# zhangyk18/GeoBi-GNN

Hardware: AMD Instinct MI355X
Metric: M-edges/s (fwd+bwd) on Synthetic set (higher is better)
Workload: dtype f32; 1 GPU; Synthetic train, batch=4 meshes (~20k faces each), fwd+bwd [BASELINE.json configs[2]]: per rank 4 noisy icospheres n=32 (F=20480) as one disjoint-union graph, L1/L1 loss, grad all-reduce + Adam step inside the timed region; ONE resident batch replayed every step, its level-0 CSR / reverse-edge index / corner lists / loss weights built in warm-up and cached per mesh (with --full, extra.fresh_batch:; meshes_per_rank=4, edges_per_rank_step=1351448, parallelism=dp1, mesh_groups_in_flight=1, split_allreduce=False, collective=none

## Files before the change

### geobi_gnn_amd/csrc/capi.hip

```cpp
#include "../../include/geobi_hip.h"

#include <stdarg.h>
#include <stdio.h>
#include <stdlib.h>

#include <mutex>
#include <vector>

#include "common.h"

namespace geobi {

static thread_local char g_err[512] = "";

int set_error(const char* fmt, ...) {
  va_list ap;
  va_start(ap, fmt);
  vsnprintf(g_err, sizeof(g_err), fmt, ap);
  va_end(ap);
  return 1;
}

struct ProfRec {
  hipEvent_t a, b;
// ... 276 lines not shown
int geobi_set_head_precision(int mode) { return set_head_precision(mode); }
int geobi_set_rowpass_form(int staged, int chunked64) { return set_rowpass_form(staged, chunked64); }
int geobi_set_column_parts(int parts) { return set_column_parts(parts); }

size_t geobi_match_coarsen_ws_bytes(int64_t N) { return match_coarsen_ws_bytes(N); }
int geobi_match_coarsen(const int32_t* rowptr, const int32_t* col, const float* w, int64_t N, int rounds, int init,
                        int32_t* state, int32_t* cluster_final, int32_t* cnew, int32_t* segptr, int32_t* members,
                        int32_t* counters, void* ws, size_t ws_bytes, void* stream) {
  SIZES(N, 0);
  NOTNULL(rowptr); NOTNULL(state); NOTNULL(cluster_final); NOTNULL(cnew); NOTNULL(segptr);
  NOTNULL(members); NOTNULL(counters); NOTNULL(ws);
  return match_coarsen(rowptr, col, w, N, rounds, init, state, cluster_final, cnew, segptr, members, counters, ws,
                       ws_bytes, S(stream));
}

size_t geobi_relabel_ws_bytes(int64_t N) { return relabel_ws_bytes(N); }
int geobi_relabel_compact(const int32_t* cluster, int64_t N, int rep_is_self, int32_t* cnew, int32_t* count,
                          void* ws, size_t ws_bytes, void* stream) {
  SIZES(N, 0);
  NOTNULL(cluster); NOTNULL(cnew); NOTNULL(count);
  return relabel_compact(cluster, N, rep_is_self, cnew, count, ws, ws_bytes, S(stream));
}

size_t geobi_segment_csr_ws_bytes(int64_t n) { return segment_csr_ws_bytes(n); }
int geobi_segment_csr(const int32_t* seg, int64_t n, int64_t nseg, int32_t* segptr, int32_t* members, void* ws,
                      size_t ws_bytes, void* stream) {
  SIZES(nseg, n);
  NOTNULL(segptr);
  return segment_csr(seg, n, nseg, segptr, members, ws, ws_bytes, S(stream));
}
// ... 373 lines not shown
```

### geobi_gnn_amd/csrc/common.h

```cpp
#pragma once
#include <hip/hip_runtime.h>
#include <stddef.h>
#include <stdint.h>

#include <atomic>

#define GEOBI_H 9
#define GEOBI_HP 12

namespace geobi {

int set_error(const char* fmt, ...);

#define GEOBI_HIP(expr)                                                                   \
  do {                                                                                    \
    hipError_t e_ = (expr);                                                               \
    if (e_ != hipSuccess)                                                                 \
      return ::geobi::set_error("%s:%d %s -> %s", __FILE__, __LINE__, #expr, hipGetErrorString(e_)); \
  } while (0)
#define GEOBI_LAUNCH_OK() GEOBI_HIP(hipGetLastError())
#define GEOBI_TRY(expr)        \
  do {                         \
    int r_ = (expr);           \
    if (r_ != 0) return r_;    \
// ... 141 lines not shown
              float* dlin_w, float* du_w, float* dc, float* dbias, int accumulate, void* ws, size_t ws_bytes,
              hipStream_t s);
struct CopySeg { const void* src; void* dst; int64_t n; int32_t add; float value; };
int concat32(const CopySeg* segs, int n_segs, int is_float, hipStream_t s);
int edge_weight_t10(const float* x, int C, const int32_t* row, const int32_t* col, const float* w_in, int64_t E,
                    float* w_out, hipStream_t s, int32_t* zero8 = nullptr);
int edge_weight_att(const float* x, int C, const float* att_l, const float* att_r, const int32_t* row, const int32_t* col,
                    const float* w_in, int64_t N, int64_t E, float* node_ws, float* w_out, hipStream_t s);
int gather_f32(const float* src, const int32_t* idx, int64_t n, float* dst, hipStream_t s);
int expand_rowptr(const int32_t* rowptr, int64_t N, int32_t* row, hipStream_t s);
size_t match_ws_bytes(int64_t N);
size_t match_coarsen_ws_bytes(int64_t N);
int match_coarsen(const int32_t* rowptr, const int32_t* col, const float* w, int64_t N, int rounds, int init,
                  int32_t* state, int32_t* cluster_final, int32_t* cnew, int32_t* segptr, int32_t* members,
                  int32_t* counters, void* ws, size_t ws_bytes, hipStream_t s, void* rowinfo_out = nullptr,
                  bool* rowinfo_made = nullptr);
int match_heavy_edge(const int32_t* rowptr, const int32_t* col, const float* w, int64_t N, int rounds, int init,
                     int32_t* cluster, int32_t* cluster_final, int32_t* status, void* ws, size_t ws_bytes, hipStream_t s);
void set_match_round_cap(int cap);
size_t relabel_ws_bytes(int64_t N);
int relabel_compact(const int32_t* cluster, int64_t N, int rep_is_self, int32_t* cnew, int32_t* count, void* ws,
                    size_t ws_bytes,
                    hipStream_t s);
size_t segment_csr_ws_bytes(int64_t n);
int segment_csr(const int32_t* seg, int64_t n, int64_t nseg, int32_t* segptr, int32_t* members, void* ws,
                size_t ws_bytes, hipStream_t s);
size_t segment_pairs_ws_bytes(int64_t nseg);
int segment_csr_pairs(const int32_t* cnew, const int32_t* raw, int64_t N, int64_t nseg, int32_t* segptr,
                      int32_t* members, void* ws, size_t ws_bytes, hipStream_t s);
int segment_csr_compose(const int32_t* segptr1, const int32_t* members1, const int32_t* segptr2,
                        const int32_t* members2, int64_t nseg2, int64_t n_fine, int32_t* segptr12,
// ... 103 lines not shown
```

### geobi_gnn_amd/csrc/executor.hip

```cpp
#include "common.h"
#include "../../include/geobi_hip.h"

#include <chrono>
#include <condition_variable>
#include <cstdlib>
#include <cstring>
#include <functional>
#include <memory>
#include <mutex>
#include <thread>
#include <vector>

namespace geobi {

namespace {

static inline void cpu_relax() {
#if defined(__x86_64__) || defined(__i386__)
  __builtin_ia32_pause();
#else
  std::this_thread::yield();
#endif
}
std::atomic<long> g_spin_cap_hits{0};

constexpr float kLeak = 0.2f;
constexpr int kRounds = 8;
constexpr int kArenaFull = GEOBI_NET_ARENA;
constexpr int kFallback = GEOBI_NET_FALLBACK;

struct Level {
  int64_t N = 0, E = 0;
  const int32_t *rowptr = nullptr, *col = nullptr, *row = nullptr;
  const int32_t* pos_rev = nullptr;
  const float* w = nullptr;
};

struct ConvSave {
  const Level* g = nullptr;
  const float *xa = nullptr, *xb = nullptr;
  int Ca = 0, Cb = 0, Cout = 0;
  float slope = 1.f;
// ... 97 lines not shown
    segptr[t] = b.take<int32_t>(P + 1); members[t] = b.take<int32_t>(P);
    rowptr_c[t] = b.take<int32_t>(P + 1); row_c[t] = b.take<int32_t>(E); col_c[t] = b.take<int32_t>(E);
    w_c[t] = b.take<float>(E);
  }
  int32_t* unpool = b.take<int32_t>(P);
  const size_t m = b.mark();
  const size_t mws = match_coarsen_ws_bytes(P), pws = pool_edge_rows_ws_bytes_onepass(P, E);
  void* ws_m = b.take<char>(mws);
  void* ws_p = b.take<char>(pws);
  if (!b.ok) return kArenaFull;
  GEOBI_TRY(edge_weight_t10(x, C, g.row, g.col, g.w, E, w10, s, counters));
  const int32_t* in_rp[2] = {g.rowptr, rowptr_c[0]};
  const int32_t* in_cl[2] = {g.col, col_c[0]};
  const int32_t* in_rw[2] = {g.row, row_c[0]};
  const float* in_w[2] = {w10, w_c[0]};
  int rounds[2] = {kRounds, kRounds};
  void* rowinfo = b.take<char>((size_t)P * 16);
  if (!b.ok) return kArenaFull;
  bool rowinfo_ok = false;
  auto run_match = [&](int t, int init) {
    return match_coarsen(in_rp[t], in_cl[t], in_w[t], P, rounds[t], init, state[t], craw[t], cnew[t], segptr[t], members[t],
                         counters + 4 * t, ws_m, mws, s, rowinfo, &rowinfo_ok);
  };
  static thread_local int32_t* pub = nullptr;
  static thread_local int pub_seq = 0;
  if (pub == nullptr) {
    GEOBI_HIP(hipHostMalloc((void**)&pub, 16 * sizeof(int32_t), hipHostMallocMapped | hipHostMallocPortable));
    for (int i = 0; i < 16; ++i) pub[i] = 0;
  }
  auto run_edges = [&](int t, bool publish) {
    int32_t* ctr = counters + 4 * t;
    return pool_edge_rows(cnew[t], segptr[t], members[t], in_rp[t], in_cl[t], in_w[t], ctr + 1, P, rowptr_c[t], row_c[t],
                          col_c[t], w_c[t], ctr + 2, ctr + 3, ws_p, pws, s, E,
                          rowinfo_ok ? rowinfo : nullptr, publish ? counters : nullptr, publish ? pub : nullptr,
                          pub_seq);
  };
  pub_seq = pub_seq >= (1 << 30) ? 1 : pub_seq + 1;
// ... 16 lines not shown
        break;
      }
      if (spins > (1l << 26)) break;
    }
    if (got) {
      for (int i = 0; i < 8; ++i) h[i] = vp[i];
    } else {
      if (spins > (1l << 26)) g_spin_cap_hits.fetch_add(1, std::memory_order_relaxed);
      GEOBI_TRY(geobi_read_i32(counters, 8, h, (void*)s));
    }
  }
  bool repaired = false;
  for (int repair = 0; repair < 12 && (h[0] || h[3] || h[4] || h[7]); ++repair) {
    repaired = true;
    const int t = (h[0] || h[3]) ? 0 : 1;
    if (h[4 * t]) {
      if (rounds[t] >= 2048) break;
      rounds[t] *= 2;
      GEOBI_TRY(run_match(t, 0));
      GEOBI_HIP(hipMemsetAsync(counters + 4 * t + 2, 0, 2 * sizeof(int32_t), s));
      GEOBI_TRY(run_edges(t, false));
    } else {
      const int64_t Et = t == 0 ? E : (int64_t)h[2];
      const size_t gws = pool_edge_ws_bytes(Et);
      const size_t mk = b.mark();
      void* ws_g = b.take<char>(gws);
      if (!b.ok) return kArenaFull;
      GEOBI_HIP(hipMemsetAsync(counters + 4 * t + 2, 0, 2 * sizeof(int32_t), s));
      GEOBI_TRY(pool_edge(cnew[t], in_rw[t], in_cl[t], in_w[t], Et, P, rowptr_c[t], row_c[t], col_c[t], w_c[t],
                          counters + 4 * t + 2, ws_g, gws, s));
// ... 508 lines not shown
  return 0;
}

extern "C" size_t geobi_abi_sizeof(int which) {
  switch (which) {
    case 0: return sizeof(geobi_net_params_t);
    case 1: return sizeof(geobi_level0_t);
    case 2: return sizeof(geobi_net_out_t);
    case 3: return sizeof(geobi_train_group_t);
    case 4: return sizeof(geobi_copy_seg_t);
    default: return 0;
  }
}

extern "C" int geobi_net_spin_cap_hits(void) { return (int)g_spin_cap_hits.load(std::memory_order_relaxed); }

extern "C" int geobi_net_train_groups(const geobi_net_params_t* prm, geobi_train_group_t* groups, int n_groups,
                                      int loss_kind_v, int loss_kind_n, float* sum_into, int64_t sum_count,
                                      void* main_stream) {
  if (!prm || !groups) return set_error("geobi_net_train_groups: null argument");
  if (n_groups < 1 || n_groups > GEOBI_MAX_GROUPS) return set_error("geobi_net_train_groups: 1..%d groups", GEOBI_MAX_GROUPS);
  if ((loss_kind_v != 0 && loss_kind_v != 1) || (loss_kind_n != 0 && loss_kind_n != 1))
    return set_error("geobi_net_train_groups: loss kinds are 0 (L1) or 1 (L2)");
  if (prm->force_depth) for (int k = 0; k < n_groups; ++k)
    if (!groups[k].depth_direction) return set_error("geobi_net_train_groups: force_depth needs depth_direction");
  for (int k = 0; k < n_groups; ++k) {
    geobi_train_group_t& g = groups[k];
    if (!g.gv || !g.gf || !g.pos_rev_v || !g.pos_rev_f || !g.x_v || !g.x_f || !g.fv || !g.y_v || !g.y_f ||
        !g.corner_segptr || !g.corner_members || !g.arena || !g.losses || !g.stream)
      return set_error("geobi_net_train_groups: null field in group %d (a group needs its OWN stream, not the null stream)", k);
// ... 66 lines not shown
```

### geobi_gnn_amd/csrc/pool.hip

```cpp
#include "common.h"

#include <cstdlib>
#include <cstring>
#include <rocprim/device/device_radix_sort.hpp>
#include <rocprim/device/device_scan.hpp>

namespace geobi {

namespace {

constexpr uint64_t kSentinel = ~0ull;

static inline int key_bits(int64_t N) {
  int b = 1;
  while ((1ll << b) <= N) ++b;
  return b;
}

__global__ __launch_bounds__(256) void edge_weight_t10_kernel(const float* __restrict__ x, int C,
                                                              const int* __restrict__ row,
                                                              const int* __restrict__ col,
                                                              const float* __restrict__ w_in, int64_t E,
                                                              float* __restrict__ w_out, int* __restrict__ zero8) {
  int64_t t = (int64_t)blockIdx.x * blockDim.x + threadIdx.x;
// ... 64 lines not shown
                                                              int64_t E, float* __restrict__ w_out) {
  const int64_t e = (int64_t)blockIdx.x * blockDim.x + threadIdx.x;
  if (e >= E) return;
  const float2 r = alr[row[e]], c = alr[col[e]];
  const float alpha = (r.x + c.y) + (c.x + r.y);
  const float sg = 1.0f / (1.0f + expf(-alpha));
  w_out[e] = w_in != nullptr ? (sg + w_in[e]) * 0.5f : sg;
}

__device__ __forceinline__ bool edge_better(float w1, int a1, int b1, float w2, int a2, int b2) {
  if (w1 != w2) return w1 > w2;
  if (a1 != a2) return a1 < a2;
  return b1 < b2;
}

template <int FIRST>
__global__ __launch_bounds__(256) void match_round_kernel(const int* __restrict__ rowptr, const int* __restrict__ col,
                                   const float* __restrict__ w, const int* __restrict__ prop_prev, int N,
                                   int* __restrict__ cluster, int* __restrict__ prop_next, int* __restrict__ status) {
  constexpr int MB = 4;
  int u = blockIdx.x * blockDim.x + threadIdx.x;
  if (FIRST != 0 && u == 0) *status = 0;
  if (u >= N) return;
  const int rs = rowptr[u], re = rowptr[u + 1];
  int cu = -1, pv = -2;
  if (FIRST != 1) cu = cluster[u];
  if (FIRST == 0) pv = prop_prev[u];
  int ppv = -2;
  if (FIRST == 0) ppv = prop_prev[pv >= 0 ? pv : u];
  int vb[MB];
  float wb[MB];
#pragma unroll
  for (int i = 0; i < MB; ++i) {
    const int e = rs + i < re ? rs + i : (re > rs ? re - 1 : 0);
    vb[i] = re > rs ? col[e] : u;
    wb[i] = (w && re > rs) ? w[e] : 1.0f;
  }
// ... 34 lines not shown
      bool free_v = true;
      if (FIRST != 1) {
        if (cv[i] >= 0) free_v = false;
        else if (FIRST == 0) {
          if (pw[i] == -1) free_v = false;
          else if (pw[i] >= 0 && ppw[i] == v) free_v = false;
        }
      }
      if (!free_v) continue;
      const float we = wb[i];
      const int a = u < v ? u : v, b = u < v ? v : u;
      if (best < 0 || edge_better(we, a, b, bw, ba, bb)) { best = v; bw = we; ba = a; bb = b; }
    }
  }
  prop_next[u] = best;
}

__global__ void match_commit_kernel(const int* __restrict__ prop, int N, int* __restrict__ cluster,
                                    int* __restrict__ remaining, int* __restrict__ final, int* __restrict__ flag,
                                    int* __restrict__ sz) {
  int u = blockIdx.x * blockDim.x + threadIdx.x;
  if (u == 0 && flag) { flag[N] = 0; sz[N] = 0; }
  if (u >= N) return;
  int st = cluster[u];
  if (st < 0) {
    int v = prop[u];
    if (v == -1) st = u;
    else if (v >= 0 && prop[v] == u) st = v;
    else atomicAdd(remaining, 1);
    if (st >= 0) cluster[u] = st;
// ... 37 lines not shown
#pragma unroll
  for (int d = 1; d < 64; d <<= 1) {
    int t = __shfl_up(inc, d, 64);
    if (lane >= d) inc += t;
  }
  if (lane == 63) s_wave[wave] = inc;
  __syncthreads();
  int off = 0, tot = 0;
#pragma unroll
  for (int w = 0; w < 4; ++w) { const int t = s_wave[w]; off += w < wave ? t : 0; tot += t; }
  __syncthreads();
  total = tot;
  return off + inc - v;
}

__global__ __launch_bounds__(256) void match_commit_scan_kernel(const int* __restrict__ prop, int N,
                                                                int* __restrict__ cluster, int* __restrict__ remaining,
                                                                int* __restrict__ final, int* __restrict__ lrank,
                                                                int* __restrict__ loffs, int* __restrict__ bt_rank,
                                                                int* __restrict__ bt_offs) {
  __shared__ int s_wave[4];
  const int u = blockIdx.x * 256 + threadIdx.x;
  int rep = 0, size = 0;
  if (u < N) {
    int st = cluster[u];
    if (st < 0) {
      int v = prop[u];
      if (v == -1) st = u;
      else if (v >= 0 && prop[v] == u) st = v;
      else atomicAdd(remaining, 1);
      if (st >= 0) cluster[u] = st;
    }
    const int fin = st < 0 ? u : (u < st ? u : st);
    final[u] = fin;
    rep = fin == u ? 1 : 0;
    size = rep ? ((st >= 0 && st != u) ? 2 : 1) : 0;
  }
  int tr, to;
  const int pr = block_exclusive_scan_256(rep, s_wave, tr);
  const int po = block_exclusive_scan_256(size, s_wave, to);
  if (u < N) { lrank[u] = pr; loffs[u] = po; }
  if (threadIdx.x == 0) { bt_rank[blockIdx.x] = tr; bt_offs[blockIdx.x] = to; }
}

__global__ __launch_bounds__(256) void match_lists_scan_kernel(const int* __restrict__ state, const int* __restrict__ final,
                                                               const int* __restrict__ lrank, const int* __restrict__ loffs,
                                                               const int* __restrict__ bt_rank, const int* __restrict__ bt_offs,
                                                               int nblocks, int N, int* __restrict__ cnew,
                                                               int* __restrict__ count, int* __restrict__ segptr,
                                                               int* __restrict__ members, const int* __restrict__ rowptr,
// ... 785 lines not shown
  gather_f32_kernel<<<cdiv(n, 256), 256, 0, s>>>(src, idx, n, dst);
  GEOBI_LAUNCH_OK();
  return 0;
}

int expand_rowptr(const int32_t* rowptr, int64_t N, int32_t* row, hipStream_t s) {
  if (N <= 0) return 0;
  expand_rowptr_kernel<<<cdiv(N, 256), 256, 0, s>>>(rowptr, (int)N, row);
  GEOBI_LAUNCH_OK();
  return 0;
}

static int g_round_cap = 0;
void set_match_round_cap(int cap) { g_round_cap = cap > 0 ? cap : 0; }

static void launch_match_rounds(const int32_t* rowptr, const int32_t* col, const float* w, int N, int rounds, int init,
                                int32_t* cluster, int32_t* status, int*& pp, int*& pn, hipStream_t s) {
  const int blocks = cdiv(N, 256);
  if (g_round_cap > 0) {
    const int64_t capped = (int64_t)g_round_cap * (rounds > 8 ? rounds / 8 : 1);
    if (capped < rounds) rounds = (int)capped;
  }
  for (int r = 0; r < rounds; ++r) {
    if (r > 0)
      match_round_kernel<0><<<blocks, 256, 0, s>>>(rowptr, col, w, pp, N, cluster, pn, status);
    else if (init)
      match_round_kernel<1><<<blocks, 256, 0, s>>>(rowptr, col, w, pp, N, cluster, pn, status);
    else
      match_round_kernel<2><<<blocks, 256, 0, s>>>(rowptr, col, w, pp, N, cluster, pn, status);
    int* t = pp; pp = pn; pn = t;
  }
}

size_t match_ws_bytes(int64_t N) { return 2 * align_up((size_t)N * sizeof(int)) + 1024; }

int match_heavy_edge(const int32_t* rowptr, const int32_t* col, const float* w, int64_t N, int rounds, int init,
                     int32_t* cluster, int32_t* cluster_final, int32_t* status, void* ws, size_t ws_bytes,
                     hipStream_t s) {
  GEOBI_REQUIRE(N > 0 && rounds > 0, "match: empty graph or no rounds");
  Arena a(ws, ws_bytes);
  int* prop0 = a.take<int>(N);
  int* prop1 = a.take<int>(N);
  GEOBI_REQUIRE(a.ok() && prop0, "match: workspace too small");
  int blocks = cdiv(N, 256);
  int* pp = prop0;
  int* pn = prop1;
  launch_match_rounds(rowptr, col, w, (int)N, rounds, init, cluster, status, pp, pn, s);
  match_commit_kernel<<<blocks, 256, 0, s>>>(pp, (int)N, cluster, status, cluster_final, nullptr, nullptr);
  GEOBI_LAUNCH_OK();
  return 0;
}

size_t match_coarsen_ws_bytes(int64_t N) {
  return match_ws_bytes(N) + 5 * align_up((size_t)(N + 1) * sizeof(int)) + 2 * scan_ws_bytes(N + 1) + 1024;
}

int match_coarsen(const int32_t* rowptr, const int32_t* col, const float* w, int64_t N, int rounds, int init,
                  int32_t* state, int32_t* cluster_final, int32_t* cnew, int32_t* segptr, int32_t* members,
                  int32_t* counters, void* ws, size_t ws_bytes, hipStream_t s, void* rowinfo_out, bool* rowinfo_made) {
  GEOBI_REQUIRE(N > 0 && rounds > 0, "match_coarsen: empty graph or no rounds");
  Arena a(ws, ws_bytes);
  int* prop0 = a.take<int>(N);
  int* prop1 = a.take<int>(N);
  int* flag = a.take<int>(N + 1);
  int* sz = a.take<int>(N + 1);
  int* rank = a.take<int>(N + 1);
  int* offs = a.take<int>(N + 1);
  size_t tb = scan_ws_bytes(N + 1);
  void* temp_a = a.take<char>(tb);
  void* temp_b = a.take<char>(tb);
  GEOBI_REQUIRE(a.ok() && prop0, "match_coarsen: workspace too small (%zu < %zu)", ws_bytes, a.off);
  const int blocks = cdiv(N, 256);
  int* pp = prop0;
  int* pn = prop1;
  launch_match_rounds(rowptr, col, w, (int)N, rounds, init, state, counters, pp, pn, s);
  static const bool scan_free = [] { const char* f = getenv("GEOBI_MATCH_SCANFREE"); return !f || atoi(f) != 0; }();
  if (scan_free && blocks <= kMaxScanBlocks) {
    int* bt_rank = rank;
    int* bt_offs = offs;
    match_commit_scan_kernel<<<blocks, 256, 0, s>>>(pp, (int)N, state, counters, cluster_final, flag, sz, bt_rank, bt_offs);
    GEOBI_LAUNCH_OK();
    match_lists_scan_kernel<<<blocks, 256, 0, s>>>(state, cluster_final, flag, sz, bt_rank, bt_offs, blocks, (int)N, cnew,
                                                   counters + 1, segptr, members, rowptr, (int4*)rowinfo_out);
    GEOBI_LAUNCH_OK();
    if (rowinfo_made) *rowinfo_made = rowinfo_out != nullptr;
    return 0;
  }
  if (rowinfo_made) *rowinfo_made = false;
  match_commit_kernel<<<blocks, 256, 0, s>>>(pp, (int)N, state, counters, cluster_final, flag, sz);
  GEOBI_LAUNCH_OK();
  if (N + 1 <= kSmallScan) {
    small_exclusive_scan2_kernel<<<1, 1024, 0, s>>>(flag, sz, rank, offs, N + 1);
    GEOBI_LAUNCH_OK();
  } else {
    GEOBI_TRY(scan_exclusive_i32(temp_a, tb, flag, rank, N + 1, s));
// ... 257 lines not shown
```

### geobi_gnn_amd/executor.py

```python
import ctypes
import os

import torch

from . import _lib as L

ENABLED = os.environ.get('GEOBI_NET_EXECUTOR', '1') == '1'
STATS = {'calls': 0, 'fallback': 0, 'arena_retry': 0}

_F = ctypes.c_void_p


class _Conv(ctypes.Structure):
    _fields_ = [('lin_w', _F), ('u_w', _F), ('c', _F), ('bias', _F)]


class _Gnn(ctypes.Structure):
    _fields_ = [('conv', _Conv * 8)]


class _Params(ctypes.Structure):
    _fields_ = [('gnn_v', _Gnn), ('gnn_f', _Gnn),
                ('fc_v1_w', _F), ('fc_v1_b', _F), ('fc_v2_w', _F), ('fc_v2_b', _F),
                ('fc_f1_w', _F), ('fc_f1_b', _F), ('fc_f2_w', _F), ('fc_f2_b', _F),
# ... 165 lines not shown
    prm, pkeep = _pack_params(net)
    _check_inputs(net, data_v, data_f, fv32, dd, pkeep)
    lib = L.lib()
    nbytes = L.size_query('geobi_net_forward_arena_bytes', lv_v.N, lv_v.E, lv_f.N, lv_f.E)
    out = _Out()
    for _ in range(2):
        arena = _arena(nbytes, dev)
        rc = lib.geobi_net_forward(ctypes.byref(prm), ctypes.byref(lv_v), ctypes.byref(lv_f), x_v.data_ptr(),
                                   x_f.data_ptr(), fv32.data_ptr(), None if dd is None else dd.data_ptr(),
                                   arena.data_ptr(), arena.numel(), ctypes.byref(out), L.stream())
        if rc != 3:
            break
        nbytes = max(2 * int(out.used_bytes), 2 * nbytes)
        STATS['arena_retry'] += 1
    STATS['calls'] += 1
    if rc == 2:
        STATS['fallback'] += 1
        return None
    if rc != 0:
        L.check(rc, 'geobi_net_forward')
    V, F = lv_v.N, lv_f.N
    verts, normals = _results(arena, out, V, F)
    key = _arena_key(dev)
    _GENERATION[key] = _GENERATION.get(key, 0) + 1
    _set_module_state(net, arena, out, (key, _GENERATION[key]))
    return verts, normals


_GENERATION = {}

# ... 76 lines not shown
    nbytes = _LEARNED.get(shape_key) or L.size_query('geobi_net_train_arena_bytes', *shape_key)
    out, handle = _Out(), ctypes.c_int64(0)
    for _ in range(4):
        arena = None
        arena = torch.empty(nbytes, dtype=torch.uint8, device=dev)
        rc = lib.geobi_net_forward_train(ctypes.byref(prm), ctypes.byref(lv_v), ctypes.byref(lv_f), gv.pos_in.data_ptr(),
                                         gf.pos_in.data_ptr(), x_v.data_ptr(), x_f.data_ptr(), fv32.data_ptr(),
                                         None if dd is None else dd.data_ptr(), arena.data_ptr(), nbytes,
                                         ctypes.byref(out), ctypes.byref(handle), L.stream())
        if rc != 3:
            break
        used = int(out.used_bytes)
        nbytes = int(1.25 * used) + (64 << 20) if used > nbytes else 2 * nbytes
        STATS['arena_retry'] += 1
    STATS['calls'] += 1
    if rc == 2:
        STATS['fallback'] += 1
        return None
    if rc != 0:
        L.check(rc, 'geobi_net_forward_train')
    _learned_size(_LEARNED, shape_key, out.used_bytes)
    STATS['train_arena_bytes'], STATS['train_need_bytes'] = nbytes, int(out.used_bytes)
    V, F = lv_v.N, lv_f.N
    verts, normals = _results(arena, out, V, F)
    _set_module_state(net, arena, out)
    return verts, normals, Recorded(handle.value, arena, keep, net, corner)


FACET_EVENTS = None

# ... 142 lines not shown
                for k, pr in enumerate(self._prep):
                    g, res = pr['g'], pr['res']
                    arena = self._arena(pr)
                    g.arena, g.arena_bytes = arena.data_ptr(), arena.numel()
                    g.grads, g.grad_flat, g.grad_count = res['gp'], res['flat'].data_ptr(), res['flat'].numel()
                    g.losses = self.losses.data_ptr() + 8 * k
                    g.stream = res['stream'].cuda_stream
                    arr[k] = g
                sig = sig[:3] + (tuple(pr['res']['arena'].data_ptr() for pr in self._prep),)
                cached = self._call = (sig, tensors, prm, arr)
            _, tensors, prm, arr = cached
            rc = lib.geobi_net_train_groups(ctypes.byref(prm), ctypes.cast(arr, ctypes.c_void_p), n,
                                            _KINDS[self.kinds[0]], _KINDS[self.kinds[1]], self.bucket.flat.data_ptr(),
                                            self.bucket.flat.numel(), L.stream())
            STATS['calls'] += 1
            if rc != 3:
                break
            STATS['arena_retry'] += 1
            for k, pr in enumerate(self._prep):
                if arr[k].rc == 3:
                    used = int(arr[k].out.used_bytes)
                    have = pr['res']['arena'].numel()
                    self._arena(pr, grow=int(1.25 * used) + (64 << 20) if used > have else 2 * have)
        if rc == 2:
            STATS['fallback'] += 1
            return self._sequential()
        if rc != 0:
            L.check(rc, 'geobi_net_train_groups')
        for k, pr in enumerate(self._prep):
            _learned_size(_LEARNED_GROUP, pr['shape'], arr[k].out.used_bytes)
# ... 27 lines not shown
```

### geobi_gnn_amd/net_util.py

```python
import os

import torch
import torch.nn.functional as F
from torch import nn

from . import _lib as L
from . import ops
from .data import Data
from .graph import Graph, graph_of, attach

MATCH_ROUNDS = 8
MATCH_ROUNDS_MAX = 2048


def _i32(t):
    return t.to(torch.int32).contiguous()


def hip_match(graph, weight_sorted, rounds=MATCH_ROUNDS, state=None, status=None):
    dev = graph.device
    init = state is None
    if init:
        state = torch.empty(graph.N, dtype=torch.int32, device=dev)
    cluster = torch.empty(graph.N, dtype=torch.int32, device=dev)
    if status is None:
        status = torch.zeros(1, dtype=torch.int32, device=dev)
    ws = L.workspace(L.size_query('geobi_match_ws_bytes', graph.N), dev)
    w = None if weight_sorted is None else weight_sorted.contiguous()
    L.call('geobi_match_heavy_edge', L.ptr(graph.rowptr_out), L.ptr(graph.col_out), L.ptr(w), graph.N, rounds,
           1 if init else 0, L.ptr(state), L.ptr(cluster), L.ptr(status), L.ptr(ws), ws.numel(), L.stream())
    return cluster, status, state


def hip_match_coarsen(graph, weight_sorted, counters, rounds=MATCH_ROUNDS, state=None):
    dev = graph.device
    init = state is None
    if init:
        state = torch.empty(graph.N, dtype=torch.int32, device=dev)
    cluster = torch.empty(graph.N, dtype=torch.int32, device=dev)
    cnew = torch.empty(graph.N, dtype=torch.int32, device=dev)
    sidx = ops.SegmentIndex(cnew, graph.N, build=False)
    ws = L.workspace(L.size_query('geobi_match_coarsen_ws_bytes', graph.N), dev)
    w = None if weight_sorted is None else weight_sorted.contiguous()
    L.call('geobi_match_coarsen', L.ptr(graph.rowptr_out), L.ptr(graph.col_out), L.ptr(w), graph.N, rounds,
           1 if init else 0, L.ptr(state), L.ptr(cluster), L.ptr(cnew), L.ptr(sidx.segptr), L.ptr(sidx.members),
           L.ptr(counters), L.ptr(ws), ws.numel(), L.stream())
    return cluster, cnew, sidx, state


def relabel(cluster32, count=None, rep_is_self=False):
    n = cluster32.shape[0]
    dev = cluster32.device
    cnew = torch.empty(n, dtype=torch.int32, device=dev)
    if count is None:
        count = torch.zeros(1, dtype=torch.int32, device=dev)
    ws = L.workspace(L.size_query('geobi_relabel_ws_bytes', n), dev)
    L.call('geobi_relabel_compact', L.ptr(cluster32), n, 1 if rep_is_self else 0, L.ptr(cnew), L.ptr(count), L.ptr(ws),
           ws.numel(), L.stream())
# ... 390 lines not shown
```

### include/geobi_hip.h

```cpp
#ifndef GEOBI_HIP_H_
#define GEOBI_HIP_H_

#include <stddef.h>
#include <stdint.h>

#ifdef __cplusplus
extern "C" {
#endif

#define GEOBI_HEADS 9
#define GEOBI_HEAD_STRIDE 12
#define GEOBI_MAX_NODES ((1 << 24) - 1)
#define GEOBI_MAX_EDGES ((1 << 28) - 1)

int geobi_version(void);
const char* geobi_last_error(void);

size_t geobi_csr_ws_bytes(int64_t E, int64_t N);
int geobi_csr_from_coo(const int64_t* seg, const int64_t* nbr, int64_t E, int64_t N, int drop_self,
                       int32_t* rowptr, int32_t* col, int32_t* eid, int32_t* bad, void* ws, size_t ws_bytes,
                       void* stream);
int geobi_csr_transpose(const int32_t* rowptr, const int32_t* col, int64_t N, int64_t Ecap, int32_t* rowptr_t,
                        int32_t* col_t, int32_t* pos_t, int32_t* inv_pos, void* ws, size_t ws_bytes, void* stream);
int geobi_csr_reverse_index(const int32_t* rowptr, const int32_t* row, const int32_t* col, int64_t E,
// ... 30 lines not shown
int geobi_set_column_parts(int parts);

int geobi_edge_weight_t10(const float* x, int C, const int32_t* row, const int32_t* col, const float* w_in,
                          int64_t E, float* w_out, void* stream);
int geobi_edge_weight_att(const float* x, int C, const float* att_l, const float* att_r, const int32_t* row,
                          const int32_t* col, const float* w_in, int64_t N, int64_t E, float* node_ws, float* w_out,
                          void* stream);
size_t geobi_match_ws_bytes(int64_t N);
int geobi_match_heavy_edge(const int32_t* rowptr, const int32_t* col, const float* w, int64_t N, int rounds,
                           int init, int32_t* cluster, int32_t* cluster_final, int32_t* status, void* ws, size_t ws_bytes, void* stream);
int geobi_set_match_round_cap(int cap);
size_t geobi_match_coarsen_ws_bytes(int64_t N);
int geobi_match_coarsen(const int32_t* rowptr, const int32_t* col, const float* w, int64_t N, int rounds, int init,
                        int32_t* state, int32_t* cluster_final, int32_t* cnew, int32_t* segptr, int32_t* members,
                        int32_t* counters, void* ws, size_t ws_bytes, void* stream);
size_t geobi_relabel_ws_bytes(int64_t N);
int geobi_relabel_compact(const int32_t* cluster, int64_t N, int rep_is_self, int32_t* cnew, int32_t* count,
                          void* ws, size_t ws_bytes, void* stream);
size_t geobi_segment_csr_ws_bytes(int64_t n);
int geobi_segment_csr(const int32_t* seg, int64_t n, int64_t nseg, int32_t* segptr, int32_t* members, void* ws,
                      size_t ws_bytes, void* stream);
size_t geobi_segment_pairs_ws_bytes(int64_t nseg);
int geobi_segment_csr_pairs(const int32_t* cnew, const int32_t* raw, int64_t N, int64_t nseg, int32_t* segptr,
                            int32_t* members, void* ws, size_t ws_bytes, void* stream);
int geobi_segment_csr_compose(const int32_t* segptr1, const int32_t* members1, const int32_t* segptr2,
                              const int32_t* members2, int64_t nseg2, int64_t n_fine, int32_t* segptr12,
                              int32_t* members12, void* ws, size_t ws_bytes, void* stream);
int geobi_segment_max_fwd(const float* x, int C, const int32_t* segptr, const int32_t* members, int64_t nseg,
                          float* out, int32_t* arg, void* stream);
int geobi_segment_max_bwd(const float* gout, const int32_t* arg, const int32_t* seg, int C, int64_t nseg,
// ... 125 lines not shown
size_t geobi_net_forward_arena_bytes(int64_t V, int64_t Ev, int64_t F, int64_t Ef);
int geobi_net_forward(const geobi_net_params_t* prm, const geobi_level0_t* gv, const geobi_level0_t* gf,
                      const float* x_v, const float* x_f, const int32_t* fv, const float* depth_direction,
                      void* arena, size_t arena_bytes, geobi_net_out_t* out, void* stream);

size_t geobi_net_train_arena_bytes(int64_t V, int64_t Ev, int64_t F, int64_t Ef);
int geobi_net_forward_train(const geobi_net_params_t* prm, const geobi_level0_t* gv, const geobi_level0_t* gf,
                            const int32_t* pos_rev_v, const int32_t* pos_rev_f, const float* x_v, const float* x_f,
                            const int32_t* fv, const float* depth_direction, void* arena, size_t arena_bytes,
                            geobi_net_out_t* out, int64_t* handle, void* stream);
int geobi_net_backward(int64_t handle, const float* g_verts, const float* g_normals, const geobi_net_params_t* grads,
                       int accumulate, const int32_t* corner_segptr, const int32_t* corner_members, void* stream);
int geobi_net_release(int64_t handle);
int geobi_net_backward_facet_events(void* ev_main, void* ev_side);
int geobi_net_spin_cap_hits(void);

#define GEOBI_MAX_GROUPS 8
typedef struct {
  const geobi_level0_t *gv, *gf;
  const int32_t *pos_rev_v, *pos_rev_f;
  const float *x_v, *x_f;
  const int32_t* fv;
  const float* depth_direction;
  const float *y_v, *y_f;
  const float *w_v, *w_f;
  float scale_v, scale_n;
  const int32_t *corner_segptr, *corner_members;
  void* arena;
  size_t arena_bytes;
  geobi_net_params_t grads;
// ... 25 lines not shown
```

Before: 325.6 M-edges/s.

## Finish heavy-edge matching tail in-block and cut default match rounds

During the last matching round, nodes that still hold a proposal are recorded in a small worklist, capped at 256. The commit-scan kernel then resolves these leftover nodes with an in-LDS iterative matching pass, using a hash table and up to 8 neighbour slots per node. This lets the default number of propose rounds drop from 8 to 6 and aims to avoid host-side repair retries that double the round count. The cost is a much larger shared-memory footprint in the commit-scan kernel, which may reduce occupancy, plus an atomic per proposing node in the last round. Counters for repairs are also added.

Result: no change. 323.7 M-edges/s (-0.6%).

```diff
diff --git a/geobi_gnn_amd/csrc/capi.hip b/geobi_gnn_amd/csrc/capi.hip
--- a/geobi_gnn_amd/csrc/capi.hip
+++ b/geobi_gnn_amd/csrc/capi.hip
@@ -314,6 +314,24 @@
                        ws_bytes, S(stream));
 }
 
+int geobi_match_coarsen_finish(const int32_t* rowptr, const int32_t* col, const float* w, int64_t N, int rounds, int init,
+                               int32_t* state, int32_t* cluster_final, int32_t* cnew, int32_t* segptr, int32_t* members,
+                               int32_t* counters, int32_t* worklist_len, void* ws, size_t ws_bytes, void* stream) {
+  SIZES(N, 0);
+  NOTNULL(rowptr); NOTNULL(state); NOTNULL(cluster_final); NOTNULL(cnew); NOTNULL(segptr);
+  NOTNULL(members); NOTNULL(counters); NOTNULL(ws);
+  return match_coarsen(rowptr, col, w, N, rounds, init, state, cluster_final, cnew, segptr, members, counters, ws,
+                       ws_bytes, S(stream), nullptr, nullptr, true, worklist_len);
+}
+int geobi_set_match_finish(int on) { set_match_finish(on); return 0; }
+int geobi_match_finish_enabled(void) { return match_finish_enabled(); }
+int geobi_match_finish_cap(void) { return match_finish_cap(); }
+int geobi_match_finish_slots(void) { return match_finish_slots(); }
+int geobi_match_finish_worklist_max(int reset) {
+  int v = 0;
+  return match_finish_worklist_max(reset, &v) == 0 ? v : -1;
+}
+
 size_t geobi_relabel_ws_bytes(int64_t N) { return relabel_ws_bytes(N); }
 int geobi_relabel_compact(const int32_t* cluster, int64_t N, int rep_is_self, int32_t* cnew, int32_t* count,
                           void* ws, size_t ws_bytes, void* stream) {
diff --git a/geobi_gnn_amd/csrc/common.h b/geobi_gnn_amd/csrc/common.h
--- a/geobi_gnn_amd/csrc/common.h
+++ b/geobi_gnn_amd/csrc/common.h
@@ -179,7 +179,12 @@
 int match_coarsen(const int32_t* rowptr, const int32_t* col, const float* w, int64_t N, int rounds, int init,
                   int32_t* state, int32_t* cluster_final, int32_t* cnew, int32_t* segptr, int32_t* members,
                   int32_t* counters, void* ws, size_t ws_bytes, hipStream_t s, void* rowinfo_out = nullptr,
-                  bool* rowinfo_made = nullptr);
+                  bool* rowinfo_made = nullptr, bool finish = false, int32_t* worklist_len = nullptr);
+void set_match_finish(int on);
+int match_finish_enabled();
+int match_finish_cap();
+int match_finish_slots();
+int match_finish_worklist_max(int reset, int* out);
 int match_heavy_edge(const int32_t* rowptr, const int32_t* col, const float* w, int64_t N, int rounds, int init,
                      int32_t* cluster, int32_t* cluster_final, int32_t* status, void* ws, size_t ws_bytes, hipStream_t s);
 void set_match_round_cap(int cap);
diff --git a/geobi_gnn_amd/csrc/executor.hip b/geobi_gnn_amd/csrc/executor.hip
--- a/geobi_gnn_amd/csrc/executor.hip
+++ b/geobi_gnn_amd/csrc/executor.hip
@@ -25,7 +25,13 @@
 std::atomic<long> g_spin_cap_hits{0};
 
 constexpr float kLeak = 0.2f;
-constexpr int kRounds = 8;
+std::atomic<long> g_pool_repairs[2];
+
+constexpr int kRoundsFinish = 6, kRoundsPlain = 8;
+static int match_rounds(bool finish) {
+  static const int env = [] { const char* f = getenv("GEOBI_MATCH_ROUNDS"); const int v = f ? atoi(f) : 0; return v > 0 && v <= 2048 ? v : 0; }();
+  return env ? env : (finish ? kRoundsFinish : kRoundsPlain);
+}
 constexpr int kArenaFull = GEOBI_NET_ARENA;
 constexpr int kFallback = GEOBI_NET_FALLBACK;
 
@@ -153,13 +159,15 @@
   const int32_t* in_cl[2] = {g.col, col_c[0]};
   const int32_t* in_rw[2] = {g.row, row_c[0]};
   const float* in_w[2] = {w10, w_c[0]};
+  const bool finish = match_finish_enabled() != 0;
+  const int kRounds = match_rounds(finish);
   int rounds[2] = {kRounds, kRounds};
   void* rowinfo = b.take<char>((size_t)P * 16);
   if (!b.ok) return kArenaFull;
   bool rowinfo_ok = false;
   auto run_match = [&](int t, int init) {
     return match_coarsen(in_rp[t], in_cl[t], in_w[t], P, rounds[t], init, state[t], craw[t], cnew[t], segptr[t], members[t],
-                         counters + 4 * t, ws_m, mws, s, rowinfo, &rowinfo_ok);
+                         counters + 4 * t, ws_m, mws, s, rowinfo, &rowinfo_ok, finish, nullptr);
   };
   static thread_local int32_t* pub = nullptr;
   static thread_local int pub_seq = 0;
@@ -206,6 +214,7 @@
   for (int repair = 0; repair < 12 && (h[0] || h[3] || h[4] || h[7]); ++repair) {
     repaired = true;
     const int t = (h[0] || h[3]) ? 0 : 1;
+    g_pool_repairs[h[4 * t] ? 0 : 1].fetch_add(1, std::memory_order_relaxed);
     if (h[4 * t]) {
       if (rounds[t] >= 2048) break;
       rounds[t] *= 2;
@@ -744,6 +753,9 @@
 }
 
 extern "C" int geobi_net_spin_cap_hits(void) { return (int)g_spin_cap_hits.load(std::memory_order_relaxed); }
+extern "C" int geobi_net_pool_repairs(int kind) {
+  return (kind == 0 || kind == 1) ? (int)g_pool_repairs[kind].load(std::memory_order_relaxed) : 0;
+}
 
 extern "C" int geobi_net_train_groups(const geobi_net_params_t* prm, geobi_train_group_t* groups, int n_groups,
                                       int loss_kind_v, int loss_kind_n, float* sum_into, int64_t sum_count,
diff --git a/geobi_gnn_amd/csrc/pool.hip b/geobi_gnn_amd/csrc/pool.hip
--- a/geobi_gnn_amd/csrc/pool.hip
+++ b/geobi_gnn_amd/csrc/pool.hip
@@ -102,13 +102,18 @@
   return b1 < b2;
 }
 
-template <int FIRST>
+constexpr int kFinishCap = 256;
+template <int FIRST, bool LIST = false>
 __global__ __launch_bounds__(256) void match_round_kernel(const int* __restrict__ rowptr, const int* __restrict__ col,
                                    const float* __restrict__ w, const int* __restrict__ prop_prev, int N,
-                                   int* __restrict__ cluster, int* __restrict__ prop_next, int* __restrict__ status) {
+                                   int* __restrict__ cluster, int* __restrict__ prop_next, int* __restrict__ status,
+                                   int* __restrict__ wl) {
   constexpr int MB = 4;
   int u = blockIdx.x * blockDim.x + threadIdx.x;
-  if (FIRST != 0 && u == 0) *status = 0;
+  if (FIRST != 0 && u == 0) {
+    *status = 0;
+    if (!LIST && wl != nullptr) wl[0] = 0;
+  }
   if (u >= N) return;
   const int rs = rowptr[u], re = rowptr[u + 1];
   int cu = -1, pv = -2;
@@ -173,6 +178,10 @@
     }
   }
   prop_next[u] = best;
+  if (LIST && best >= 0) {
+    const int i = atomicAdd(wl, 1);
+    if (i < kFinishCap) wl[1 + i] = u;
+  }
 }
 
 __global__ void match_commit_kernel(const int* __restrict__ prop, int N, int* __restrict__ cluster,
@@ -240,26 +249,146 @@
   return off + inc - v;
 }
 
+constexpr int kFinishSlots = 8;
+constexpr int kFinishRowMax = 1024;
+constexpr int kFinishHash = 512;
+static_assert(kFinishCap <= 256, "one worklist node per thread of a 256-thread block");
+
+struct FinishLds {
+  int id[kFinishCap];
+  int st[kFinishCap];
+  int pr[kFinishCap];
+  int tab[kFinishHash];
+  float nw[kFinishCap * kFinishSlots];
+  unsigned char nj[kFinishCap * kFinishSlots];
+  int fail;
+};
+__device__ int g_finish_wl_max = 0;
+
+__device__ __forceinline__ int finish_hash(int u) { return (int)(((unsigned)u * 2654435761u) >> 23) & (kFinishHash - 1); }
+
+__device__ __forceinline__ int finish_lookup(const FinishLds& L, int v) {
+  int h = finish_hash(v);
+  for (int i = 0; i < kFinishHash; ++i) {
+    const int sl = L.tab[h];
+    if (sl < 0) return -1;
+    if (L.id[sl] == v) return sl;
+    h = (h + 1) & (kFinishHash - 1);
+  }
+  return -1;
+}
+
+__device__ bool finish_tail(FinishLds& L, int cnt, int wu, const int* __restrict__ prop,
+                            const int* __restrict__ rowptr, const int* __restrict__ col, const float* __restrict__ w) {
+  const int t = threadIdx.x;
+  for (int i = t; i < kFinishHash; i += 256) L.tab[i] = -1;
+  if (t == 0) L.fail = 0;
+  bool fr = false;
+  int rs = 0, re = 0;
+  if (t < cnt) {
+    const int wp = prop[wu];
+    rs = rowptr[wu]; re = rowptr[wu + 1];
+    const int wpp = wp >= 0 ? prop[wp] : -2;
+    fr = wp >= 0 && wpp != wu;
+    L.id[t] = wu;
+    L.st[t] = fr ? -1 : (wp >= 0 ? wp : wu);
+  }
+  __syncthreads();
+  if (t < cnt) {
+    int h = finish_hash(wu);
+    for (int i = 0; i < kFinishHash; ++i) {
+      if (atomicCAS(&L.tab[h], -1, t) == -1) break;
+      h = (h + 1) & (kFinishHash - 1);
+    }
+  }
+  if (__syncthreads_count(fr) == 0) return false;
+  int deg = 0;
+  if (fr) {
+    if (re - rs > kFinishRowMax) deg = kFinishSlots + 1;
+    for (int e = rs; e < re && deg <= kFinishSlots; ++e) {
+      const int v = col[e];
+      if (v == wu) continue;
+      const int j = finish_lookup(L, v);
+      if (j < 0 || L.st[j] != -1) continue;
+      if (deg < kFinishSlots) {
+        L.nj[t * kFinishSlots + deg] = (unsigned char)j;
+        L.nw[t * kFinishSlots + deg] = w ? w[e] : 1.0f;
+      }
+      ++deg;
+    }
+    if (deg > kFinishSlots) L.fail = 1;
+  }
+  __syncthreads();
+  if (L.fail) return false;
+  for (int it = 0; it < kFinishCap; ++it) {
+    int best = -1, ba = 0, bb = 0;
+    float bw = 0.f;
+    if (fr) {
+      for (int k = 0; k < deg; ++k) {
+        const int j = L.nj[t * kFinishSlots + k];
+        if (L.st[j] != -1) continue;
+        const int v = L.id[j];
+        const float we = L.nw[t * kFinishSlots + k];
+        const int a = wu < v ? wu : v, b = wu < v ? v : wu;
+        if (best < 0 || edge_better(we, a, b, bw, ba, bb)) { best = j; bw = we; ba = a; bb = b; }
+      }
+      L.pr[t] = best;
+    }
+    __syncthreads();
+    if (fr) {
+      if (best < 0) { L.st[t] = wu; fr = false; }
+      else if (L.pr[best] == t) { L.st[t] = L.id[best]; fr = false; }
+    }
+    if (__syncthreads_count(fr) == 0) break;
+  }
+  return true;
+}
+
+template <bool FIN>
 __global__ __launch_bounds__(256) void match_commit_scan_kernel(const int* __restrict__ prop, int N,
                                                                 int* __restrict__ cluster, int* __restrict__ remaining,
                                                                 int* __restrict__ final, int* __restrict__ lrank,
                                                                 int* __restrict__ loffs, int* __restrict__ bt_rank,
-                                                                int* __restrict__ bt_offs) {
+                                                                int* __restrict__ bt_offs, const int* __restrict__ wl,
+                                                                const int* __restrict__ rowptr,
+                                                                const int* __restrict__ col, const float* __restrict__ w,
+                                                                int* __restrict__ wl_len) {
   __shared__ int s_wave[4];
+  __shared__ FinishLds s_fin;
   const int u = blockIdx.x * 256 + threadIdx.x;
+  const int cnt = FIN ? wl[0] : 0;
+  const int wu = FIN ? wl[1 + threadIdx.x] : -1;
+  int st = -1, v = -2, pv = -2;
+  if (u < N) {
+    st = cluster[u];
+    v = prop[u];
+    if (v >= 0) pv = prop[v];
+  }
+  bool fin = false;
+  if (FIN) {
+    if (cnt > 0 && cnt <= kFinishCap) fin = finish_tail(s_fin, cnt, wu, prop, rowptr, col, w);
+    if (u == 0) {
+      if (wl_len != nullptr) *wl_len = cnt;
+      if (cnt > 0) atomicMax(&g_finish_wl_max, cnt);
+    }
+  }
   int rep = 0, size = 0;
   if (u < N) {
-    int st = cluster[u];
     if (st < 0) {
-      int v = prop[u];
       if (v == -1) st = u;
-      else if (v >= 0 && prop[v] == u) st = v;
-      else atomicAdd(remaining, 1);
+      else if (v >= 0 && pv == u) st = v;
+      else {
+        if (FIN && fin) {
+          const int j = finish_lookup(s_fin, u);
+          if (j >= 0) st = s_fin.st[j];
+        }
+        if (st < 0) atomicAdd(remaining, 1);
+      }
       if (st >= 0) cluster[u] = st;
     }
-    const int fin = st < 0 ? u : (u < st ? u : st);
-    final[u] = fin;
-    rep = fin == u ? 1 : 0;
+    const int fin_id = st < 0 ? u : (u < st ? u : st);
+    final[u] = fin_id;
+    rep = fin_id == u ? 1 : 0;
     size = rep ? ((st >= 0 && st != u) ? 2 : 1) : 0;
   }
   int tr, to;
@@ -1075,22 +1204,45 @@
 static int g_round_cap = 0;
 void set_match_round_cap(int cap) { g_round_cap = cap > 0 ? cap : 0; }
 
-static void launch_match_rounds(const int32_t* rowptr, const int32_t* col, const float* w, int N, int rounds, int init,
-                                int32_t* cluster, int32_t* status, int*& pp, int*& pn, hipStream_t s) {
+static int g_match_finish = [] { const char* f = getenv("GEOBI_MATCH_FINISH"); return (!f || atoi(f) != 0) ? 1 : 0; }();
+void set_match_finish(int on) { g_match_finish = on ? 1 : 0; }
+int match_finish_enabled() { return g_match_finish; }
+int match_finish_cap() { return kFinishCap; }
+int match_finish_slots() { return kFinishSlots; }
+int match_finish_worklist_max(int reset, int* out) {
+  int v = 0;
+  GEOBI_HIP(hipMemcpyFromSymbol(&v, HIP_SYMBOL(g_finish_wl_max), sizeof(int)));
+  if (reset) {
+    const int z = 0;
+    GEOBI_HIP(hipMemcpyToSymbol(HIP_SYMBOL(g_finish_wl_max), &z, sizeof(int)));
+  }
+  *out = v;
+  return 0;
+}
+
+static int launch_match_rounds(const int32_t* rowptr, const int32_t* col, const float* w, int N, int rounds, int init,
+                               int32_t* cluster, int32_t* status, int*& pp, int*& pn, hipStream_t s, int* wl = nullptr) {
   const int blocks = cdiv(N, 256);
   if (g_round_cap > 0) {
     const int64_t capped = (int64_t)g_round_cap * (rounds > 8 ? rounds / 8 : 1);
     if (capped < rounds) rounds = (int)capped;
   }
+  if (wl != nullptr && rounds == 1) GEOBI_HIP(hipMemsetAsync(wl, 0, sizeof(int), s));
   for (int r = 0; r < rounds; ++r) {
-    if (r > 0)
-      match_round_kernel<0><<<blocks, 256, 0, s>>>(rowptr, col, w, pp, N, cluster, pn, status);
-    else if (init)
-      match_round_kernel<1><<<blocks, 256, 0, s>>>(rowptr, col, w, pp, N, cluster, pn, status);
-    else
-      match_round_kernel<2><<<blocks, 256, 0, s>>>(rowptr, col, w, pp, N, cluster, pn, status);
+    const bool list = wl != nullptr && r == rounds - 1;
+    if (r > 0) {
+      if (list) match_round_kernel<0, true><<<blocks, 256, 0, s>>>(rowptr, col, w, pp, N, cluster, pn, status, wl);
+      else match_round_kernel<0><<<blocks, 256, 0, s>>>(rowptr, col, w, pp, N, cluster, pn, status, wl);
+    } else if (init) {
+      if (list) match_round_kernel<1, true><<<blocks, 256, 0, s>>>(rowptr, col, w, pp, N, cluster, pn, status, wl);
+      else match_round_kernel<1><<<blocks, 256, 0, s>>>(rowptr, col, w, pp, N, cluster, pn, status, wl);
+    } else {
+      if (list) match_round_kernel<2, true><<<blocks, 256, 0, s>>>(rowptr, col, w, pp, N, cluster, pn, status, wl);
+      else match_round_kernel<2><<<blocks, 256, 0, s>>>(rowptr, col, w, pp, N, cluster, pn, status, wl);
+    }
     int* t = pp; pp = pn; pn = t;
   }
+  return 0;
 }
 
 size_t match_ws_bytes(int64_t N) { return 2 * align_up((size_t)N * sizeof(int)) + 1024; }
@@ -1106,19 +1258,21 @@
   int blocks = cdiv(N, 256);
   int* pp = prop0;
   int* pn = prop1;
-  launch_match_rounds(rowptr, col, w, (int)N, rounds, init, cluster, status, pp, pn, s);
+  GEOBI_TRY(launch_match_rounds(rowptr, col, w, (int)N, rounds, init, cluster, status, pp, pn, s));
   match_commit_kernel<<<blocks, 256, 0, s>>>(pp, (int)N, cluster, status, cluster_final, nullptr, nullptr);
   GEOBI_LAUNCH_OK();
   return 0;
 }
 
 size_t match_coarsen_ws_bytes(int64_t N) {
-  return match_ws_bytes(N) + 5 * align_up((size_t)(N + 1) * sizeof(int)) + 2 * scan_ws_bytes(N + 1) + 1024;
+  return match_ws_bytes(N) + 5 * align_up((size_t)(N + 1) * sizeof(int)) + 2 * scan_ws_bytes(N + 1) + 1024 +
+         align_up((size_t)(kFinishCap + 1) * sizeof(int));
 }
 
 int match_coarsen(const int32_t* rowptr, const int32_t* col, const float* w, int64_t N, int rounds, int init,
                   int32_t* state, int32_t* cluster_final, int32_t* cnew, int32_t* segptr, int32_t* members,
-                  int32_t* counters, void* ws, size_t ws_bytes, hipStream_t s, void* rowinfo_out, bool* rowinfo_made) {
+                  int32_t* counters, void* ws, size_t ws_bytes, hipStream_t s, void* rowinfo_out, bool* rowinfo_made,
+                  bool finish, int32_t* worklist_len) {
   GEOBI_REQUIRE(N > 0 && rounds > 0, "match_coarsen: empty graph or no rounds");
   Arena a(ws, ws_bytes);
   int* prop0 = a.take<int>(N);
@@ -1130,16 +1284,24 @@
   size_t tb = scan_ws_bytes(N + 1);
   void* temp_a = a.take<char>(tb);
   void* temp_b = a.take<char>(tb);
+  int* wl = a.take<int>(kFinishCap + 1);
   GEOBI_REQUIRE(a.ok() && prop0, "match_coarsen: workspace too small (%zu < %zu)", ws_bytes, a.off);
   const int blocks = cdiv(N, 256);
   int* pp = prop0;
   int* pn = prop1;
-  launch_match_rounds(rowptr, col, w, (int)N, rounds, init, state, counters, pp, pn, s);
   static const bool scan_free = [] { const char* f = getenv("GEOBI_MATCH_SCANFREE"); return !f || atoi(f) != 0; }();
+  finish = finish && scan_free && blocks <= kMaxScanBlocks;
+  GEOBI_TRY(launch_match_rounds(rowptr, col, w, (int)N, rounds, init, state, counters, pp, pn, s, finish ? wl : nullptr));
+  if (!finish && worklist_len != nullptr) GEOBI_HIP(hipMemsetAsync(worklist_len, 0, sizeof(int32_t), s));
   if (scan_free && blocks <= kMaxScanBlocks) {
     int* bt_rank = rank;
     int* bt_offs = offs;
-    match_commit_scan_kernel<<<blocks, 256, 0, s>>>(pp, (int)N, state, counters, cluster_final, flag, sz, bt_rank, bt_offs);
+    if (finish)
+      match_commit_scan_kernel<true><<<blocks, 256, 0, s>>>(pp, (int)N, state, counters, cluster_final, flag, sz, bt_rank,
+                                                            bt_offs, wl, rowptr, col, w, worklist_len);
+    else
+      match_commit_scan_kernel<false><<<blocks, 256, 0, s>>>(pp, (int)N, state, counters, cluster_final, flag, sz, bt_rank,
+                                                             bt_offs, nullptr, nullptr, nullptr, nullptr, nullptr);
     GEOBI_LAUNCH_OK();
     match_lists_scan_kernel<<<blocks, 256, 0, s>>>(state, cluster_final, flag, sz, bt_rank, bt_offs, blocks, (int)N, cnew,
                                                    counters + 1, segptr, members, rowptr, (int4*)rowinfo_out);
diff --git a/geobi_gnn_amd/executor.py b/geobi_gnn_amd/executor.py
--- a/geobi_gnn_amd/executor.py
+++ b/geobi_gnn_amd/executor.py
@@ -7,6 +7,11 @@
 
 ENABLED = os.environ.get('GEOBI_NET_EXECUTOR', '1') == '1'
 STATS = {'calls': 0, 'fallback': 0, 'arena_retry': 0}
+
+
+def _mirror_repairs(lib):
+    STATS['pool_repairs_undecided'] = lib.geobi_net_pool_repairs(0)
+    STATS['pool_repairs_wide'] = lib.geobi_net_pool_repairs(1)
 
 _F = ctypes.c_void_p
 
@@ -203,6 +208,7 @@
         nbytes = max(2 * int(out.used_bytes), 2 * nbytes)
         STATS['arena_retry'] += 1
     STATS['calls'] += 1
+    _mirror_repairs(lib)
     if rc == 2:
         STATS['fallback'] += 1
         return None
@@ -309,6 +315,7 @@
         nbytes = int(1.25 * used) + (64 << 20) if used > nbytes else 2 * nbytes
         STATS['arena_retry'] += 1
     STATS['calls'] += 1
+    _mirror_repairs(lib)
     if rc == 2:
         STATS['fallback'] += 1
         return None
@@ -481,6 +488,7 @@
                                             _KINDS[self.kinds[0]], _KINDS[self.kinds[1]], self.bucket.flat.data_ptr(),
                                             self.bucket.flat.numel(), L.stream())
             STATS['calls'] += 1
+            _mirror_repairs(lib)
             if rc != 3:
                 break
             STATS['arena_retry'] += 1
diff --git a/geobi_gnn_amd/net_util.py b/geobi_gnn_amd/net_util.py
--- a/geobi_gnn_amd/net_util.py
+++ b/geobi_gnn_amd/net_util.py
@@ -32,7 +32,7 @@
     return cluster, status, state
 
 
-def hip_match_coarsen(graph, weight_sorted, counters, rounds=MATCH_ROUNDS, state=None):
+def hip_match_coarsen(graph, weight_sorted, counters, rounds=MATCH_ROUNDS, state=None, worklist_len=None):
     dev = graph.device
     init = state is None
     if init:
@@ -42,6 +42,11 @@
     sidx = ops.SegmentIndex(cnew, graph.N, build=False)
     ws = L.workspace(L.size_query('geobi_match_coarsen_ws_bytes', graph.N), dev)
     w = None if weight_sorted is None else weight_sorted.contiguous()
+    if worklist_len is not None:
+        L.call('geobi_match_coarsen_finish', L.ptr(graph.rowptr_out), L.ptr(graph.col_out), L.ptr(w), graph.N, rounds,
+               1 if init else 0, L.ptr(state), L.ptr(cluster), L.ptr(cnew), L.ptr(sidx.segptr), L.ptr(sidx.members),
+               L.ptr(counters), L.ptr(worklist_len), L.ptr(ws), ws.numel(), L.stream())
+        return cluster, cnew, sidx, state
     L.call('geobi_match_coarsen', L.ptr(graph.rowptr_out), L.ptr(graph.col_out), L.ptr(w), graph.N, rounds,
            1 if init else 0, L.ptr(state), L.ptr(cluster), L.ptr(cnew), L.ptr(sidx.segptr), L.ptr(sidx.members),
            L.ptr(counters), L.ptr(ws), ws.numel(), L.stream())
diff --git a/include/geobi_hip.h b/include/geobi_hip.h
--- a/include/geobi_hip.h
+++ b/include/geobi_hip.h
@@ -68,6 +68,14 @@
 int geobi_match_coarsen(const int32_t* rowptr, const int32_t* col, const float* w, int64_t N, int rounds, int init,
                         int32_t* state, int32_t* cluster_final, int32_t* cnew, int32_t* segptr, int32_t* members,
                         int32_t* counters, void* ws, size_t ws_bytes, void* stream);
+int geobi_match_coarsen_finish(const int32_t* rowptr, const int32_t* col, const float* w, int64_t N, int rounds, int init,
+                               int32_t* state, int32_t* cluster_final, int32_t* cnew, int32_t* segptr, int32_t* members,
+                               int32_t* counters, int32_t* worklist_len, void* ws, size_t ws_bytes, void* stream);
+int geobi_set_match_finish(int on);
+int geobi_match_finish_enabled(void);
+int geobi_match_finish_cap(void);
+int geobi_match_finish_slots(void);
+int geobi_match_finish_worklist_max(int reset);
 size_t geobi_relabel_ws_bytes(int64_t N);
 int geobi_relabel_compact(const int32_t* cluster, int64_t N, int rep_is_self, int32_t* cnew, int32_t* count,
                           void* ws, size_t ws_bytes, void* stream);
@@ -223,6 +231,7 @@
 int geobi_net_release(int64_t handle);
 int geobi_net_backward_facet_events(void* ev_main, void* ev_side);
 int geobi_net_spin_cap_hits(void);
+int geobi_net_pool_repairs(int kind);
 
 #define GEOBI_MAX_GROUPS 8
 typedef struct {
```
